# MichSchli/RelationPrediction

Measured on NVIDIA H100. Metric: R-GCN layer fwd+bwd M-edges/sec, higher is better.
Workload: dtype f32

## Files before the change

### relationprediction_b200/csrc/gemm_tf32x3.cu

```cuda
#include <cuda_runtime.h>
#include <stdint.h>

#include <algorithm>
#include <string>

#include "kernels.cuh"

namespace {

constexpr int BM = 128, BN = 128, BK = 32;
constexpr int STAGES = 3;
template <int NST, int TBN>
struct StageShape {
  static constexpr int STAGE_COUNT = NST;
  static constexpr int A_PLANE = BM * BK * 4;
  static constexpr int B_PLANE = TBN * BK * 4;
  static constexpr int BYTES = 2 * A_PLANE + 2 * B_PLANE;
  static constexpr int FRAG = TBN / 2;
};
using NtStage = StageShape<STAGES, BN>;
constexpr int TILE_BYTES = NtStage::A_PLANE;
constexpr int STAGE_BYTES = NtStage::BYTES;
constexpr int SMEM_BYTES = STAGES * STAGE_BYTES + 1024;
constexpr int N_PRODUCERS = 128;
constexpr int N_CONSUMERS = 256;
constexpr int N_THREADS = N_PRODUCERS + N_CONSUMERS;
constexpr int N_FRAG = BN / 2;
static_assert(BM == BN, "the producers use one row schedule for both operands");

__device__ __forceinline__ uint32_t smem_u32(const void* p) {
  return (uint32_t)__cvta_generic_to_shared(p);
}
__device__ __forceinline__ void mbar_init(uint64_t* bar, uint32_t count) {
  asm volatile("mbarrier.init.shared::cta.b64 [%0], %1;" ::"r"(smem_u32(bar)), "r"(count));
}
__device__ __forceinline__ void mbar_arrive(uint64_t* bar) {
  asm volatile("mbarrier.arrive.shared::cta.b64 _, [%0];" ::"r"(smem_u32(bar)) : "memory");
}
__device__ __forceinline__ void mbar_wait(uint64_t* bar, uint32_t parity) {
  asm volatile(
      "{\n\t"
      ".reg .pred p;\n\t"
      "WAIT_LOOP:\n\t"
      "mbarrier.try_wait.parity.shared::cta.b64 p, [%0], %1;\n\t"
      "@p bra WAIT_DONE;\n\t"
      "bra WAIT_LOOP;\n\t"
      "WAIT_DONE:\n\t"
      "}" ::"r"(smem_u32(bar)),
      "r"(parity)
      : "memory");
}
__device__ __forceinline__ void cp_async16(uint32_t dst, const void* src, uint32_t src_bytes) {
  asm volatile("cp.async.cg.shared.global [%0], [%1], 16, %2;" ::"r"(dst), "l"(src), "r"(src_bytes)
               : "memory");
}

__device__ __forceinline__ uint64_t make_desc(uint32_t smem_addr) {
  return (uint64_t)((smem_addr & 0x3FFFFu) >> 4) | (1ull << 16) | ((uint64_t)(1024 >> 4) << 32) | (1ull << 62);
}

__device__ __forceinline__ void wgmma_tf32(float (&d)[64], uint64_t da, uint64_t db, uint32_t accumulate) {
  asm volatile(
      "{\n\t"
      ".reg .pred p;\n\t"
      "setp.ne.b32 p, %66, 0;\n\t"
      "wgmma.mma_async.sync.aligned.m64n128k8.f32.tf32.tf32 "
      "{%0, %1, %2, %3, %4, %5, %6, %7, %8, %9, %10, %11, %12, %13, %14, %15, %16, %17, %18, %19, %20, %21, %22, "
      "%23, %24, %25, %26, %27, %28, %29, %30, %31, %32, %33, %34, %35, %36, %37, %38, %39, %40, %41, %42, %43, %44, "
      "%45, %46, %47, %48, %49, %50, %51, %52, %53, %54, %55, %56, %57, %58, %59, %60, %61, %62, %63}, "
      "%64, %65, p, 1, 1;\n\t"
      "}"
      : "+f"(d[0]), "+f"(d[1]), "+f"(d[2]), "+f"(d[3]), "+f"(d[4]), "+f"(d[5]), "+f"(d[6]), "+f"(d[7]),
        "+f"(d[8]), "+f"(d[9]), "+f"(d[10]), "+f"(d[11]), "+f"(d[12]), "+f"(d[13]), "+f"(d[14]), "+f"(d[15]),
        "+f"(d[16]), "+f"(d[17]), "+f"(d[18]), "+f"(d[19]), "+f"(d[20]), "+f"(d[21]), "+f"(d[22]), "+f"(d[23]),
        "+f"(d[24]), "+f"(d[25]), "+f"(d[26]), "+f"(d[27]), "+f"(d[28]), "+f"(d[29]), "+f"(d[30]), "+f"(d[31]),
        "+f"(d[32]), "+f"(d[33]), "+f"(d[34]), "+f"(d[35]), "+f"(d[36]), "+f"(d[37]), "+f"(d[38]), "+f"(d[39]),
        "+f"(d[40]), "+f"(d[41]), "+f"(d[42]), "+f"(d[43]), "+f"(d[44]), "+f"(d[45]), "+f"(d[46]), "+f"(d[47]),
        "+f"(d[48]), "+f"(d[49]), "+f"(d[50]), "+f"(d[51]), "+f"(d[52]), "+f"(d[53]), "+f"(d[54]), "+f"(d[55]),
        "+f"(d[56]), "+f"(d[57]), "+f"(d[58]), "+f"(d[59]), "+f"(d[60]), "+f"(d[61]), "+f"(d[62]), "+f"(d[63])
      : "l"(da), "l"(db), "r"(accumulate)
      : "memory");
}
__device__ __forceinline__ void wgmma_tf32(float (&d)[32], uint64_t da, uint64_t db, uint32_t accumulate) {
  asm volatile(
      "{\n\t"
      ".reg .pred p;\n\t"
      "setp.ne.b32 p, %34, 0;\n\t"
      "wgmma.mma_async.sync.aligned.m64n64k8.f32.tf32.tf32 "
      "{%0, %1, %2, %3, %4, %5, %6, %7, %8, %9, %10, %11, %12, %13, %14, %15, %16, %17, %18, %19, %20, %21, %22, "
      "%23, %24, %25, %26, %27, %28, %29, %30, %31}, "
      "%32, %33, p, 1, 1;\n\t"
      "}"
      : "+f"(d[0]), "+f"(d[1]), "+f"(d[2]), "+f"(d[3]), "+f"(d[4]), "+f"(d[5]), "+f"(d[6]), "+f"(d[7]),
        "+f"(d[8]), "+f"(d[9]), "+f"(d[10]), "+f"(d[11]), "+f"(d[12]), "+f"(d[13]), "+f"(d[14]), "+f"(d[15]),
        "+f"(d[16]), "+f"(d[17]), "+f"(d[18]), "+f"(d[19]), "+f"(d[20]), "+f"(d[21]), "+f"(d[22]), "+f"(d[23]),
        "+f"(d[24]), "+f"(d[25]), "+f"(d[26]), "+f"(d[27]), "+f"(d[28]), "+f"(d[29]), "+f"(d[30]), "+f"(d[31])
      : "l"(da), "l"(db), "r"(accumulate)
      : "memory");
}
template <int NF>
__device__ __forceinline__ void fence_acc(float (&d)[NF]) {
#pragma unroll
  for (int i = 0; i < NF; ++i) asm volatile("" : "+f"(d[i])::"memory");
}

__device__ __forceinline__ void split_tf32_trunc(float a, float& hi, float& lo) {
  hi = __uint_as_float(__float_as_uint(a) & 0xffffe000u);
  lo = __uint_as_float(__float_as_uint(a - hi) & 0xffffe000u);
}
__device__ __forceinline__ void split_tf32(float a, float& hi, float& lo) {
  uint32_t h, l;
  asm("cvt.rna.tf32.f32 %0, %1;" : "=r"(h) : "f"(a));
  hi = __uint_as_float(h);
  asm("cvt.rna.tf32.f32 %0, %1;" : "=r"(l) : "f"(a - hi));
  lo = __uint_as_float(l);
}

__device__ __forceinline__ uint32_t swz(int r, int c) {
  return (uint32_t)((r >> 3) * 1024 + (r & 7) * 128 + ((c ^ (r & 7)) << 4));
}

template <int NST = STAGES>
__device__ __forceinline__ void init_barriers(uint64_t* full_bar, uint64_t* empty_bar) {
  for (int s = 0; s < NST; ++s) {
    mbar_init(&full_bar[s], N_PRODUCERS);
    mbar_init(&empty_bar[s], N_CONSUMERS);
  }
  asm volatile("fence.mbarrier_init.release.cluster;" ::: "memory");
}

template <class S>
__device__ __forceinline__ void consume_tile(uint32_t smem_base, uint64_t* full_bar, uint64_t* empty_bar, int g0,
                                             int num_kb, uint32_t a_rows, float (&big)[S::FRAG],
                                             float (&small)[S::FRAG]) {
  for (int kb = 0; kb < num_kb; ++kb) {
    const int g = g0 + kb;
    const int s = g % S::STAGE_COUNT;
    mbar_wait(&full_bar[s], (uint32_t)(g / S::STAGE_COUNT) & 1u);
    const uint32_t a_hi = smem_base + s * S::BYTES + a_rows, a_lo = a_hi + S::A_PLANE;
    const uint32_t b_hi = smem_base + s * S::BYTES + 2 * S::A_PLANE, b_lo = b_hi + S::B_PLANE;
    asm volatile("wgmma.fence.sync.aligned;" ::: "memory");
#pragma unroll
    for (int kk = 0; kk < BK / 8; ++kk) {
      const uint64_t dah = make_desc(a_hi + kk * 32), dal = make_desc(a_lo + kk * 32);
      const uint64_t dbh = make_desc(b_hi + kk * 32), dbl = make_desc(b_lo + kk * 32);
      const uint32_t acc = (kb == 0 && kk == 0) ? 0u : 1u;
      wgmma_tf32(small, dal, dbh, acc);
      wgmma_tf32(small, dah, dbl, 1u);
      wgmma_tf32(big, dah, dbh, acc);
    }
    asm volatile("wgmma.commit_group.sync.aligned;" ::: "memory");
    asm volatile("wgmma.wait_group.sync.aligned 0;" ::: "memory");
    fence_acc(big);
    fence_acc(small);
    mbar_arrive(&empty_bar[s]);
  }
}

struct TileCtx {
  int tile;
  int m0, n0;
  int r0, c0;
  int M, N;
  int lane, warp;
};

__device__ __forceinline__ uint32_t col_bit(uint32_t word, int col) { return (word >> (col & 31)) & 1u; }
template <int NF, class Fn>
__device__ __forceinline__ void for_each_col(const TileCtx& t, int h, const uint32_t* bits, int words, Fn fn) {
  const int row = t.r0 + 8 * h;
#pragma unroll
  for (int cb = 0; cb < NF / 16; ++cb) {
    const int chunk = t.n0 + 32 * cb;
    const uint32_t w =
        (bits && row < t.M && chunk < t.N) ? __ldg(bits + (size_t)row * words + (chunk >> 5)) : 0u;
#pragma unroll
    for (int jj = 0; jj < 4; ++jj) {
#pragma unroll
      for (int e = 0; e < 2; ++e) {
        const int j = 4 * cb + jj, col = t.c0 + 8 * j + e;
        fn(4 * j + 2 * h + e, 2 * j + e, col, w);
      }
    }
  }
}
template <class Fn>
__device__ __forceinline__ void for_each_pair(const TileCtx& t, int h, Fn fn) {
#pragma unroll
  for (int j = 0; j < BN / 8; ++j) {
    const int col = t.c0 + 8 * j;
    if (col < t.N) fn(4 * j + 2 * h, col);
  }
}
__device__ __forceinline__ void rank_counts_flush(int raw, int kn, int row, int M, int32_t* raw_cnt,
                                                  int32_t* known_cnt, int lane) {
  raw += __shfl_xor_sync(0xffffffffu, raw, 1);
  raw += __shfl_xor_sync(0xffffffffu, raw, 2);
  kn += __shfl_xor_sync(0xffffffffu, kn, 1);
  kn += __shfl_xor_sync(0xffffffffu, kn, 2);
  if ((lane & 3) == 0 && row < M) {
    if (raw) atomicAdd(raw_cnt + row, raw);
    if (kn) atomicAdd(known_cnt + row, kn);
  }
}
__device__ __forceinline__ void warp_part_store(float x, float* part, const TileCtx& t) {
#pragma unroll
  for (int o = 16; o > 0; o >>= 1) x += __shfl_xor_sync(0xffffffffu, x, o);
  if (t.lane == 0) part[(size_t)t.tile * 8 + t.warp] = x;
}
__device__ __forceinline__ float sigmoid_ref(float x) { return 1.0f / (1.0f + expf(-x)); }

struct StoreEpi {
  float* C;
  int64_t ldc;
  int accumulate;

  __device__ __forceinline__ void operator()(const TileCtx& t, const float (&big)[N_FRAG],
                                             const float (&small)[N_FRAG]) const {
#pragma unroll
    for (int h = 0; h < 2; ++h) {
      const int row = t.r0 + 8 * h;
      if (row >= t.M) continue;
      float* crow = C + (size_t)row * ldc;
      for_each_pair(t, h, [&](int r, int col) {
        float2 o = make_float2(big[r] + small[r], big[r + 1] + small[r + 1]);
        if (accumulate) {
          const float2 old = *reinterpret_cast<const float2*>(crow + col);
          o.x += old.x;
          o.y += old.y;
        }
        *reinterpret_cast<float2*>(crow + col) = o;
      });
    }
  }
};

struct RankEpi {
  const float* gold_sig;
  const int32_t* gold_col;
// ... 137 lines not shown
            bc[h] = oc;
          }
        }
        if (bi >= 0 && bc[h] == mine) left[h] &= ~(1u << bi);
      }
      if (!__any_sync(0xffffffffu, bc[0] != 0x7fffffff || bc[1] != 0x7fffffff)) break;
      if (writer) {
#pragma unroll
        for (int h = 0; h < 2; ++h)
          if (r0 + 8 * h < M)
            *slot(h, p) = bc[h] == 0x7fffffff ? none : make_uint2(__float_as_uint(be[h]), (uint32_t)bc[h]);
      }
    }
    if (writer) {
      for (; p < k; ++p) {
#pragma unroll
        for (int h = 0; h < 2; ++h)
          if (r0 + 8 * h < M) *slot(h, p) = none;
      }
    }
  }
};

struct BceEpi {
  const uint32_t* labels;
  int words;
  float pos, neg;
  float scale;
  const float* g_scale;
  float* Gt;
  int64_t ldgt;
  float* loss_part;

  __device__ __forceinline__ void operator()(const TileCtx& t, const float (&big)[N_FRAG],
                                             const float (&small)[N_FRAG]) const {
    const float gs = scale * (g_scale ? __ldg(g_scale) : 1.f);
    float ls = 0.f;
#pragma unroll
    for (int h = 0; h < 2; ++h) {
      const int row = t.r0 + 8 * h;
      if (row >= t.M) continue;
      for_each_col<N_FRAG>(t, h, labels, words, [&](int r, int, int col, uint32_t word) {
        if (col < t.N) {
          const float z = big[r] + small[r];
          const float y = col_bit(word, col) ? pos : neg;
          ls += fmaxf(z, 0.f) - z * y + log1pf(expf(-fabsf(z)));
          if (Gt) Gt[(size_t)col * ldgt + row] = (1.0f / (1.0f + expf(-z)) - y) * gs;
        }
      });
    }
    warp_part_store(ls, loss_part, t);
  }
};

enum : int { EPI_STORE = 0, EPI_RANK = 1, EPI_HIGHWAY = 2, EPI_VAR = 3, EPI_TOPK = 4, EPI_BCE = 5 };
template <int EPI>
struct Epilogue;
template <> struct Epilogue<EPI_STORE> { using type = StoreEpi; };
template <> struct Epilogue<EPI_RANK> { using type = RankEpi; };
template <> struct Epilogue<EPI_HIGHWAY> { using type = HighwayEpi; };
template <> struct Epilogue<EPI_VAR> { using type = VarEpi; };
template <> struct Epilogue<EPI_TOPK> { using type = TopKEpi; };
template <> struct Epilogue<EPI_BCE> { using type = BceEpi; };

template <int EPI>
__global__ void __launch_bounds__(N_THREADS, 1)
    k_gemm_tf32x3(const float* __restrict__ A, int64_t lda, const float* __restrict__ Bhi,
                  const float* __restrict__ Blo, int64_t ldb, int M, int N, int K, int n_tiles,
                  const typename Epilogue<EPI>::type epi) {
  extern __shared__ uint8_t smem_raw[];
  __shared__ __align__(8) uint64_t full_bar[STAGES], empty_bar[STAGES];

  const uint32_t smem_base = (smem_u32(smem_raw) + 1023u) & ~1023u;
  const int tid = threadIdx.x, lane = tid & 31;
  const int tn = (N + BN - 1) / BN;
  const int num_kb = (K + BK - 1) / BK;
  const int n_mine = (n_tiles - (int)blockIdx.x + (int)gridDim.x - 1) / (int)gridDim.x;
  const int total_g = n_mine * num_kb;

  if (tid == 0) init_barriers(full_bar, empty_bar);
  __syncthreads();

  if (tid < N_PRODUCERS) {
    const int c = tid & 7;
    const int rbase = tid >> 3;
    const uint32_t soff = swz(rbase, c);
    constexpr int NR = BM / 16;

    int b_kb = 0, b_tile = (int)blockIdx.x, b_stage = 0;
    size_t b_off = 0;
    uint32_t b_ok = 0;
    auto b_set_tile = [&]() {
      const int r0 = (b_tile % tn) * BN + rbase;
      b_ok = 0;
#pragma unroll
      for (int i = 0; i < NR; ++i) b_ok |= (r0 + 16 * i < N ? 1u : 0u) << i;
      b_off = (b_ok & 1u) ? (size_t)r0 * ldb + c * 4 : 0;
    };
    b_set_tile();
    auto issue_b = [&]() {
      const uint32_t b_hi = smem_base + b_stage * STAGE_BYTES + 2 * TILE_BYTES + soff, b_lo = b_hi + TILE_BYTES;
      const bool col_ok = b_kb * BK + c * 4 < K;
      const size_t kof = b_off + (size_t)b_kb * BK;
#pragma unroll
      for (int i = 0; i < NR; ++i) {
        const bool ok = col_ok && ((b_ok >> i) & 1u);
        const size_t o = kof + (size_t)(16 * i) * ldb;
        cp_async16(b_hi + 2048 * i, ok ? Bhi + o : Bhi, ok ? 16u : 0u);
        cp_async16(b_lo + 2048 * i, ok ? Blo + o : Blo, ok ? 16u : 0u);
      }
      asm volatile("cp.async.commit_group;" ::: "memory");
      b_stage = b_stage + 1 == STAGES ? 0 : b_stage + 1;
      if (++b_kb == num_kb) {
        b_kb = 0;
        b_tile += (int)gridDim.x;
        b_set_tile();
      }
    };
    int a_kb = 0, a_tile = (int)blockIdx.x;
    size_t a_off = 0;
    uint32_t a_ok = 0;
    auto a_set_tile = [&]() {
      const int r0 = (a_tile / tn) * BM + rbase;
      a_ok = 0;
#pragma unroll
      for (int i = 0; i < NR; ++i) a_ok |= (r0 + 16 * i < M ? 1u : 0u) << i;
      a_off = (a_ok & 1u) ? (size_t)r0 * lda + c * 4 : 0;
    };
    a_set_tile();
    auto load_a = [&](float4 (&v)[NR]) {
      const bool col_ok = a_kb * BK + c * 4 < K;
      const float* p = A + a_off + (size_t)a_kb * BK;
#pragma unroll
      for (int i = 0; i < NR; ++i)
        v[i] = (col_ok && ((a_ok >> i) & 1u)) ? __ldg(reinterpret_cast<const float4*>(p + (size_t)(16 * i) * lda))
                                               : make_float4(0.f, 0.f, 0.f, 0.f);
      if (++a_kb == num_kb) {
        a_kb = 0;
        a_tile += (int)gridDim.x;
        a_set_tile();
      }
    };
    constexpr int PF = 2;
    float4 vbuf[PF + 1][NR];
    mbar_wait(&empty_bar[0], 1u);
    issue_b();
    for (int p = 0; p < PF; ++p)
      if (p < total_g) load_a(vbuf[p]);
    int s = 0;
    uint32_t ph_next = 0;
    for (int g0 = 0; g0 < total_g; g0 += PF + 1) {
#pragma unroll
      for (int u = 0; u <= PF; ++u) {
        const int g = g0 + u;
        if (g >= total_g) break;
        const bool more = g + 1 < total_g;
        const int s1 = s + 1 == STAGES ? 0 : s + 1;
        if (s1 == 0) ph_next ^= 1u;
        if (more) {
          mbar_wait(&empty_bar[s1], ph_next ^ 1u);
          issue_b();
        }
        if (g + PF < total_g) load_a(vbuf[(u + PF) % (PF + 1)]);
        const uint32_t a_hi = smem_base + s * STAGE_BYTES + soff, a_lo = a_hi + TILE_BYTES;
#pragma unroll
        for (int i = 0; i < NR; ++i) {
          float4 hi, lo;
          split_tf32_trunc(vbuf[u][i].x, hi.x, lo.x);
          split_tf32_trunc(vbuf[u][i].y, hi.y, lo.y);
          split_tf32_trunc(vbuf[u][i].z, hi.z, lo.z);
          split_tf32_trunc(vbuf[u][i].w, hi.w, lo.w);
          asm volatile("st.shared.v4.f32 [%0], {%1, %2, %3, %4};" ::"r"(a_hi + 2048 * i), "f"(hi.x), "f"(hi.y),
                       "f"(hi.z), "f"(hi.w)
                       : "memory");
          asm volatile("st.shared.v4.f32 [%0], {%1, %2, %3, %4};" ::"r"(a_lo + 2048 * i), "f"(lo.x), "f"(lo.y),
                       "f"(lo.z), "f"(lo.w)
                       : "memory");
        }
        if (more)
          asm volatile("cp.async.wait_group 1;" ::: "memory");
        else
          asm volatile("cp.async.wait_group 0;" ::: "memory");
        asm volatile("fence.proxy.async.shared::cta;" ::: "memory");
        mbar_arrive(&full_bar[s]);
        s = s1;
      }
    }
  } else {
    const int ctid = tid - N_PRODUCERS;
    const int wg = ctid >> 7, warp = ctid >> 5;
    const uint32_t a_rows = (uint32_t)(wg * 64 * 128);
    float big[N_FRAG], small[N_FRAG];
    for (int ti = 0; ti < n_mine; ++ti) {
      const int tile = (int)blockIdx.x + ti * (int)gridDim.x;
      const int m0 = (tile / tn) * BM, n0 = (tile % tn) * BN;
      consume_tile<NtStage>(smem_base, full_bar, empty_bar, ti * num_kb, num_kb, a_rows, big, small);
      const int r0 = m0 + wg * 64 + (warp & 3) * 16 + (lane >> 2), c0 = n0 + 2 * (lane & 3);
      const TileCtx t{tile, m0, n0, r0, c0, M, N, lane, warp};
      epi(t, big, small);
    }
  }
}

constexpr int TN_FLUSH_KB = 32;
constexpr int TN_STAGES = 2;
using TnStage = StageShape<TN_STAGES, BN>;
constexpr int TN_RAW = 3;
constexpr int RAW_TILE_BYTES = BK * BM * 4;
constexpr int RAW_BYTES = 2 * RAW_TILE_BYTES;
constexpr int TN_SMEM_BYTES = TN_STAGES * STAGE_BYTES + TN_RAW * RAW_BYTES + 1024;
static_assert(TN_SMEM_BYTES <= 227 * 1024, "TN kernel exceeds the shared memory of a block");
static_assert(N_PRODUCERS == 128 && BK == 32 && BM == 128, "the TN producer's lane mapping assumes these");

__device__ __forceinline__ float4 ld_shared_v4(uint32_t addr) {
  float4 v;
  asm volatile("ld.shared.v4.f32 {%0, %1, %2, %3}, [%4];" : "=f"(v.x), "=f"(v.y), "=f"(v.z), "=f"(v.w) : "r"(addr)
               : "memory");
  return v;
}
__device__ __forceinline__ void st_shared_v4(uint32_t addr, float x, float y, float z, float w) {
  asm volatile("st.shared.v4.f32 [%0], {%1, %2, %3, %4};" ::"r"(addr), "f"(x), "f"(y), "f"(z), "f"(w) : "memory");
}

__global__ void __launch_bounds__(N_THREADS, 1)
    k_gemm_tn_tf32x3(const float* __restrict__ A, int64_t lda, const float* __restrict__ B, int64_t ldb,
                     float* __restrict__ C, int64_t ldc, int M, int N, int K, int kb_per_split) {
  extern __shared__ uint8_t smem_raw[];
  __shared__ __align__(8) uint64_t full_bar[TN_STAGES], empty_bar[TN_STAGES];
  const uint32_t smem_base = (smem_u32(smem_raw) + 1023u) & ~1023u;
  const int tid = threadIdx.x, warp = tid >> 5, lane = tid & 31;
  const int tm = (M + BM - 1) / BM, tiles = tm * ((N + BN - 1) / BN);
  const int tile = (int)blockIdx.x % tiles, split = (int)blockIdx.x / tiles;
  const int m0 = (tile % tm) * BM, n0 = (tile / tm) * BN;
  const int kb_begin = split * kb_per_split;
  const int num_kb = min(kb_per_split, (K + BK - 1) / BK - kb_begin);

  if (tid == 0) init_barriers<TN_STAGES>(full_bar, empty_bar);
  __syncthreads();

  if (tid < N_PRODUCERS) {
    const uint32_t raw_base = smem_base + TN_STAGES * STAGE_BYTES;
    const bool a_ok = m0 + 4 * lane < M, b_ok = n0 + 4 * lane < N;
    const float* pa = A + (a_ok ? m0 + 4 * lane : 0);
    const float* pb = B + (b_ok ? n0 + 4 * lane : 0);
    auto issue = [&](int kbi) {
      const uint32_t dst = raw_base + (kbi % TN_RAW) * RAW_BYTES;
      const int k0 = (kb_begin + kbi) * BK + warp;
#pragma unroll
      for (int i = 0; i < 8; ++i) {
        const bool kok = k0 + 4 * i < K;
        const size_t row = kok ? (size_t)(k0 + 4 * i) : 0;
        const uint32_t off = (uint32_t)((warp + 4 * i) * 512 + ((lane ^ i) << 4));
        cp_async16(dst + off, pa + row * lda, kok && a_ok ? 16u : 0u);
        cp_async16(dst + RAW_TILE_BYTES + off, pb + row * ldb, kok && b_ok ? 16u : 0u);
      }
      asm volatile("cp.async.commit_group;" ::: "memory");
    };
    const int g = lane & 7;
    auto convert = [&](uint32_t raw, uint32_t hi_plane) {
#pragma unroll
      for (int u = 0; u < 2; ++u) {
        const int h = (lane >> 3) + 4 * warp + 16 * u;
        float4 v[4];
#pragma unroll
        for (int j = 0; j < 4; ++j) v[j] = ld_shared_v4(raw + (4 * g + j) * 512 + ((h ^ g) << 4));
        const float x[4][4] = {{v[0].x, v[1].x, v[2].x, v[3].x}, {v[0].y, v[1].y, v[2].y, v[3].y},
                               {v[0].z, v[1].z, v[2].z, v[3].z}, {v[0].w, v[1].w, v[2].w, v[3].w}};
#pragma unroll
        for (int i = 0; i < 4; ++i) {
          float hi[4], lo[4];
#pragma unroll
          for (int j = 0; j < 4; ++j) split_tf32_trunc(x[i][j], hi[j], lo[j]);
          const uint32_t a = hi_plane + swz(4 * h + i, g);
          st_shared_v4(a, hi[0], hi[1], hi[2], hi[3]);
          st_shared_v4(a + TILE_BYTES, lo[0], lo[1], lo[2], lo[3]);
        }
      }
    };
    issue(0);
    if (num_kb > 1)
      issue(1);
    else
      asm volatile("cp.async.commit_group;" ::: "memory");
    for (int kb = 0; kb < num_kb; ++kb) {
      asm volatile("cp.async.wait_group 1;" ::: "memory");
      asm volatile("bar.sync 1, %0;" ::"n"(N_PRODUCERS) : "memory");
      if (kb + 2 < num_kb)
        issue(kb + 2);
      else
        asm volatile("cp.async.commit_group;" ::: "memory");
      const int s = kb % TN_STAGES;
      mbar_wait(&empty_bar[s], ((uint32_t)(kb / TN_STAGES) & 1u) ^ 1u);
      const uint32_t raw = raw_base + (kb % TN_RAW) * RAW_BYTES, stage = smem_base + s * STAGE_BYTES;
      convert(raw, stage);
      convert(raw + RAW_TILE_BYTES, stage + 2 * TILE_BYTES);
      asm volatile("fence.proxy.async.shared::cta;" ::: "memory");
      mbar_arrive(&full_bar[s]);
    }
  } else {
    const int ctid = tid - N_PRODUCERS;
    const int wg = ctid >> 7;
    const int r0 = m0 + wg * 64 + ((ctid >> 5) & 3) * 16 + (lane >> 2);
    const int c0 = n0 + 2 * (lane & 3);
    float* const cbase = C + (size_t)r0 * ldc + c0;
    float big[N_FRAG], small[N_FRAG];
    for (int kc = 0; kc < num_kb; kc += TN_FLUSH_KB) {
      consume_tile<TnStage>(smem_base, full_bar, empty_bar, kc, min(TN_FLUSH_KB, num_kb - kc),
                            (uint32_t)(wg * 64 * 128), big, small);
      float* cp = cbase;
      asm volatile("" : "+l"(cp));
#pragma unroll
      for (int h = 0; h < 2; ++h) {
        if (r0 + 8 * h >= M) continue;
        float* crow = cp + (size_t)(8 * h) * ldc;
#pragma unroll
        for (int j = 0; j < BN / 8; ++j) {
          if (c0 + 8 * j < N)
            asm volatile("red.global.add.v2.f32 [%0], {%1, %2};" ::"l"(crow + 8 * j),
                         "f"(big[4 * j + 2 * h] + small[4 * j + 2 * h]),
                         "f"(big[4 * j + 2 * h + 1] + small[4 * j + 2 * h + 1])
                         : "memory");
        }
      }
    }
  }
}

__global__ void k_split_b(const float* __restrict__ B, int64_t ldb, int N, int K, int transposed,
                          float* __restrict__ hi, float* __restrict__ lo) {
  const int64_t total = (int64_t)N * K;
  for (int64_t i = blockIdx.x * (int64_t)blockDim.x + threadIdx.x; i < total;
       i += (int64_t)gridDim.x * blockDim.x) {
    const int n = (int)(i / K), k = (int)(i % K);
    const float v = transposed ? __ldg(B + (size_t)k * ldb + n) : __ldg(B + (size_t)n * ldb + k);
    float h, l;
    split_tf32(v, h, l);
    hi[i] = h;
    lo[i] = l;
  }
}

__global__ void k_split_b_interleave(const float* __restrict__ Wmu, const float* __restrict__ Wsig, int d, int w,
                                     int transposed, float* __restrict__ hi, float* __restrict__ lo) {
  const int64_t total = (int64_t)2 * d * w;
  const int K = transposed ? d : 2 * w;
  for (int64_t i = blockIdx.x * (int64_t)blockDim.x + threadIdx.x; i < total;
       i += (int64_t)gridDim.x * blockDim.x) {
    const int n = (int)(i / K), k = (int)(i % K);
    const int row = transposed ? k : n, c = transposed ? n : k;
    const float v = __ldg(((c & 1) ? Wsig : Wmu) + (size_t)row * w + (c >> 1));
    float h, l;
    split_tf32(v, h, l);
    hi[i] = h;
    lo[i] = l;
  }
}

constexpr int EN_BN = 64;
constexpr int EN_STAGES = 4;
constexpr int EN_LOOKAHEAD = 2;
using EnsStage = StageShape<EN_STAGES, EN_BN>;
constexpr int EN_Q_BYTES = EnsStage::A_PLANE;
constexpr int EN_C_BYTES = EnsStage::B_PLANE;
constexpr int EN_STAGE_BYTES = EnsStage::BYTES;
constexpr int EN_SMEM_BYTES = EN_STAGES * EN_STAGE_BYTES + 1024;
constexpr int EN_FRAG = EnsStage::FRAG;
static_assert(EN_SMEM_BYTES <= 227 * 1024, "ensemble kernel exceeds the shared memory of a block");
static_assert(EN_LOOKAHEAD < EN_STAGES, "the lookahead needs a free stage");

struct EnsMember {
  const float* q_hi;
  const float* q_lo;
  const float* c_hi;
  const float* c_lo;
  const float* gold_sig;
  int K;
};
struct EnsEpi {
  EnsMember a, b;
  double w, omw;
  const int32_t* gold_col;
  const uint32_t* known;
  int words;
  int32_t* raw_cnt;
  int32_t* known_cnt;
};

__global__ void __launch_bounds__(N_THREADS, 1)
    k_gemm_ensemble_rank(int M, int N, int n_tiles, EnsEpi re) {
  extern __shared__ uint8_t smem_raw[];
  __shared__ __align__(8) uint64_t full_bar[EN_STAGES], empty_bar[EN_STAGES];
  const uint32_t smem_base = (smem_u32(smem_raw) + 1023u) & ~1023u;
  const int tid = threadIdx.x, lane = tid & 31;
  const int tn = (N + EN_BN - 1) / EN_BN;
  const int nkb_a = (re.a.K + BK - 1) / BK, nkb_b = (re.b.K + BK - 1) / BK, nkb = nkb_a + nkb_b;
  const int n_mine = (n_tiles - (int)blockIdx.x + (int)gridDim.x - 1) / (int)gridDim.x;
  const int total_g = n_mine * nkb;

  if (tid == 0) init_barriers<EN_STAGES>(full_bar, empty_bar);
  __syncthreads();

  if (tid < N_PRODUCERS) {
    const int c = tid & 7;
    const int rbase = tid >> 3;
    const uint32_t soff = swz(rbase, c);
    int i_tile = (int)blockIdx.x, i_kb = 0, stage = 0;
    auto issue = [&]() {
      const bool mb = i_kb >= nkb_a;
      const float* qh = mb ? re.b.q_hi : re.a.q_hi;
      const float* ql = mb ? re.b.q_lo : re.a.q_lo;
      const float* ch = mb ? re.b.c_hi : re.a.c_hi;
      const float* cl = mb ? re.b.c_lo : re.a.c_lo;
      const int K = mb ? re.b.K : re.a.K;
      const int k = (mb ? i_kb - nkb_a : i_kb) * BK + c * 4;
      const bool col_ok = k < K;
      const int m0 = (i_tile / tn) * BM, n0 = (i_tile % tn) * EN_BN;
      const uint32_t st = smem_base + stage * EN_STAGE_BYTES + soff;
#pragma unroll
      for (int i = 0; i < BM / 16; ++i) {
        const int row = m0 + rbase + 16 * i;
        const bool ok = col_ok && row < M;
        const size_t o = ok ? (size_t)row * K + k : 0;
        cp_async16(st + 2048 * i, qh + o, ok ? 16u : 0u);
        cp_async16(st + EN_Q_BYTES + 2048 * i, ql + o, ok ? 16u : 0u);
      }
#pragma unroll
      for (int i = 0; i < EN_BN / 16; ++i) {
        const int row = n0 + rbase + 16 * i;
        const bool ok = col_ok && row < N;
        const size_t o = ok ? (size_t)row * K + k : 0;
        cp_async16(st + 2 * EN_Q_BYTES + 2048 * i, ch + o, ok ? 16u : 0u);
        cp_async16(st + 2 * EN_Q_BYTES + EN_C_BYTES + 2048 * i, cl + o, ok ? 16u : 0u);
      }
      asm volatile("cp.async.commit_group;" ::: "memory");
      stage = stage + 1 == EN_STAGES ? 0 : stage + 1;
      if (++i_kb == nkb) {
        i_kb = 0;
        i_tile += (int)gridDim.x;
      }
    };
    for (int g = 0; g < EN_LOOKAHEAD; ++g) {
      if (g < total_g) {
        mbar_wait(&empty_bar[g % EN_STAGES], ((uint32_t)(g / EN_STAGES) & 1u) ^ 1u);
        issue();
      } else {
        asm volatile("cp.async.commit_group;" ::: "memory");
      }
    }
    for (int g = 0; g < total_g; ++g) {
      const int gn = g + EN_LOOKAHEAD;
      if (gn < total_g) {
        mbar_wait(&empty_bar[gn % EN_STAGES], ((uint32_t)(gn / EN_STAGES) & 1u) ^ 1u);
        issue();
      } else {
        asm volatile("cp.async.commit_group;" ::: "memory");
      }
      asm volatile("cp.async.wait_group %0;" ::"n"(EN_LOOKAHEAD) : "memory");
      asm volatile("fence.proxy.async.shared::cta;" ::: "memory");
      mbar_arrive(&full_bar[g % EN_STAGES]);
    }
  } else {
    const int ctid = tid - N_PRODUCERS;
    const int wg = ctid >> 7, warp = ctid >> 5;
    const uint32_t a_rows = (uint32_t)(wg * 64 * 128);
    float big_a[EN_FRAG], small_a[EN_FRAG], big_b[EN_FRAG], small_b[EN_FRAG];
    for (int ti = 0; ti < n_mine; ++ti) {
      const int tile = (int)blockIdx.x + ti * (int)gridDim.x;
      const int m0 = (tile / tn) * BM, n0 = (tile % tn) * EN_BN;
      consume_tile<EnsStage>(smem_base, full_bar, empty_bar, ti * nkb, nkb_a, a_rows, big_a, small_a);
      consume_tile<EnsStage>(smem_base, full_bar, empty_bar, ti * nkb + nkb_a, nkb_b, a_rows, big_b, small_b);
      const int r0 = m0 + wg * 64 + (warp & 3) * 16 + (lane >> 2), c0 = n0 + 2 * (lane & 3);
      const TileCtx t{tile, m0, n0, r0, c0, M, N, lane, warp};
#pragma unroll
      for (int h = 0; h < 2; ++h) {
        const int row = t.r0 + 8 * h;
        int raw = 0, kn = 0;
        if (row < M) {
          const double G = __dadd_rn(__dmul_rn(re.w, (double)__ldg(re.a.gold_sig + row)),
                                     __dmul_rn(re.omw, (double)__ldg(re.b.gold_sig + row)));
          const int gold_c = __ldg(re.gold_col + row);
          for_each_col<EN_FRAG>(t, h, re.known, re.words, [&](int r, int, int col, uint32_t word) {
            const float sa = sigmoid_ref(big_a[r] + small_a[r]);
            const float sb = sigmoid_ref(big_b[r] + small_b[r]);
            const double cv = __dadd_rn(__dmul_rn(re.w, (double)sa), __dmul_rn(re.omw, (double)sb));
            if (col < N && (cv >= G || col == gold_c)) {
              ++raw;
              kn += (int)col_bit(word, col);
            }
          });
        }
        rank_counts_flush(raw, kn, row, M, re.raw_cnt, re.known_cnt, lane);
      }
    }
  }
}

__global__ void k_split_trunc(float* __restrict__ a, float* __restrict__ lo, int64_t count4) {
  for (int64_t i = blockIdx.x * (int64_t)blockDim.x + threadIdx.x; i < count4; i += (int64_t)gridDim.x * blockDim.x) {
    float4 v = reinterpret_cast<float4*>(a)[i], h, l;
    split_tf32_trunc(v.x, h.x, l.x);
    split_tf32_trunc(v.y, h.y, l.y);
    split_tf32_trunc(v.z, h.z, l.z);
    split_tf32_trunc(v.w, h.w, l.w);
    reinterpret_cast<float4*>(a)[i] = h;
    reinterpret_cast<float4*>(lo)[i] = l;
  }
}

}

static int sm_count() {
  int dev = 0, sms = 132;
  cudaGetDevice(&dev);
  cudaDeviceGetAttribute(&sms, cudaDevAttrMultiProcessorCount, dev);
  return sms;
}

static int64_t tiles_of(int64_t M, int64_t N, int bn) { return ((M + BM - 1) / BM) * ((N + bn - 1) / bn); }

template <auto Kernel, class... Args>
static int launch_persistent(const char* what, const char* label, int smem, int64_t tiles, int64_t tile_limit,
                             cudaStream_t st, Args... args) {
  static bool attr_set = false;
  if (!attr_set) {
    int rc = rgcn_check_cuda(cudaFuncSetAttribute(Kernel, cudaFuncAttributeMaxDynamicSharedMemorySize, smem),
                             (std::string("cudaFuncSetAttribute(") + label + " smem)").c_str());
    if (rc) return rc;
    attr_set = true;
  }
  if (tiles > tile_limit) {
    rgcn_set_error(std::string(what) + ": too many tiles");
    return RGCN_ERR_INVALID;
  }
  const unsigned grid = (unsigned)std::min<int64_t>(tiles, sm_count());
  Kernel<<<grid, N_THREADS, smem, st>>>(args...);
  ++g_rgcn_launches;
  return rgcn_check_cuda(cudaGetLastError(), label);
}
constexpr int64_t TILE_LIMIT = 0x7fffffffLL;
constexpr int64_t PART_TILE_LIMIT = TILE_LIMIT / 8;

template <int EPI>
static int launch_nt(const char* what, const char* label, int64_t tile_limit, cudaStream_t st, const float* A,
                     int64_t lda, const float* Bt_hi, const float* Bt_lo, int64_t ldb, int M, int N, int K,
                     const typename Epilogue<EPI>::type& epi) {
  const int64_t tiles = tiles_of(M, N, BN);
  return launch_persistent<k_gemm_tf32x3<EPI>>(what, label, SMEM_BYTES, tiles, tile_limit, st, A, lda, Bt_hi, Bt_lo,
                                               ldb, M, N, K, (int)tiles, epi);
}

static int split_blocks(int64_t items) { return (int)std::min<int64_t>((items + 255) / 256, 132 * 8); }

int launch_gemm_split_b(const float* B, int64_t ldb, int N, int K, int transposed, float* hi, float* lo,
// ... 163 lines not shown
```

Baseline: 129.2.

## Feed WGMMA A operand from registers with consumer-side split and deeper pipelining

```diff
diff --git a/relationprediction_b200/csrc/gemm_tf32x3.cu b/relationprediction_b200/csrc/gemm_tf32x3.cu
--- a/relationprediction_b200/csrc/gemm_tf32x3.cu
+++ b/relationprediction_b200/csrc/gemm_tf32x3.cu
@@ -9,24 +9,28 @@
 namespace {
 
 constexpr int BM = 128, BN = 128, BK = 32;
-constexpr int STAGES = 3;
-template <int NST, int TBN>
+constexpr int STAGES = 4;
+template <int NST, int TBN, int A_PLANES>
 struct StageShape {
   static constexpr int STAGE_COUNT = NST;
   static constexpr int A_PLANE = BM * BK * 4;
+  static constexpr int A_BYTES = A_PLANES * A_PLANE;
   static constexpr int B_PLANE = TBN * BK * 4;
-  static constexpr int BYTES = 2 * A_PLANE + 2 * B_PLANE;
+  static constexpr int BYTES = A_BYTES + 2 * B_PLANE;
   static constexpr int FRAG = TBN / 2;
 };
-using NtStage = StageShape<STAGES, BN>;
+using NtStage = StageShape<STAGES, BN, 1>;
 constexpr int TILE_BYTES = NtStage::A_PLANE;
 constexpr int STAGE_BYTES = NtStage::BYTES;
 constexpr int SMEM_BYTES = STAGES * STAGE_BYTES + 1024;
+static_assert(SMEM_BYTES <= 227 * 1024, "NT kernel exceeds the shared memory of a block");
 constexpr int N_PRODUCERS = 128;
 constexpr int N_CONSUMERS = 256;
 constexpr int N_THREADS = N_PRODUCERS + N_CONSUMERS;
 constexpr int N_FRAG = BN / 2;
-static_assert(BM == BN, "the producers use one row schedule for both operands");
+constexpr int NT_PRODUCER_REGS = 40, TN_PRODUCER_REGS = 56;
+template <int PRODUCER_REGS>
+constexpr int CONSUMER_REGS = (168 * N_THREADS - N_PRODUCERS * PRODUCER_REGS) / N_CONSUMERS / 8 * 8;
 
 __device__ __forceinline__ uint32_t smem_u32(const void* p) {
   return (uint32_t)__cvta_generic_to_shared(p);
@@ -59,16 +63,16 @@
   return (uint64_t)((smem_addr & 0x3FFFFu) >> 4) | (1ull << 16) | ((uint64_t)(1024 >> 4) << 32) | (1ull << 62);
 }
 
-__device__ __forceinline__ void wgmma_tf32(float (&d)[64], uint64_t da, uint64_t db, uint32_t accumulate) {
+__device__ __forceinline__ void wgmma_tf32(float (&d)[64], const uint32_t (&a)[4], uint64_t db, uint32_t accumulate) {
   asm volatile(
       "{\n\t"
       ".reg .pred p;\n\t"
-      "setp.ne.b32 p, %66, 0;\n\t"
+      "setp.ne.b32 p, %69, 0;\n\t"
       "wgmma.mma_async.sync.aligned.m64n128k8.f32.tf32.tf32 "
       "{%0, %1, %2, %3, %4, %5, %6, %7, %8, %9, %10, %11, %12, %13, %14, %15, %16, %17, %18, %19, %20, %21, %22, "
       "%23, %24, %25, %26, %27, %28, %29, %30, %31, %32, %33, %34, %35, %36, %37, %38, %39, %40, %41, %42, %43, %44, "
       "%45, %46, %47, %48, %49, %50, %51, %52, %53, %54, %55, %56, %57, %58, %59, %60, %61, %62, %63}, "
-      "%64, %65, p, 1, 1;\n\t"
+      "{%64, %65, %66, %67}, %68, p, 1, 1;\n\t"
       "}"
       : "+f"(d[0]), "+f"(d[1]), "+f"(d[2]), "+f"(d[3]), "+f"(d[4]), "+f"(d[5]), "+f"(d[6]), "+f"(d[7]),
         "+f"(d[8]), "+f"(d[9]), "+f"(d[10]), "+f"(d[11]), "+f"(d[12]), "+f"(d[13]), "+f"(d[14]), "+f"(d[15]),
@@ -78,24 +82,24 @@
         "+f"(d[40]), "+f"(d[41]), "+f"(d[42]), "+f"(d[43]), "+f"(d[44]), "+f"(d[45]), "+f"(d[46]), "+f"(d[47]),
         "+f"(d[48]), "+f"(d[49]), "+f"(d[50]), "+f"(d[51]), "+f"(d[52]), "+f"(d[53]), "+f"(d[54]), "+f"(d[55]),
         "+f"(d[56]), "+f"(d[57]), "+f"(d[58]), "+f"(d[59]), "+f"(d[60]), "+f"(d[61]), "+f"(d[62]), "+f"(d[63])
-      : "l"(da), "l"(db), "r"(accumulate)
+      : "r"(a[0]), "r"(a[1]), "r"(a[2]), "r"(a[3]), "l"(db), "r"(accumulate)
       : "memory");
 }
-__device__ __forceinline__ void wgmma_tf32(float (&d)[32], uint64_t da, uint64_t db, uint32_t accumulate) {
+__device__ __forceinline__ void wgmma_tf32(float (&d)[32], const uint32_t (&a)[4], uint64_t db, uint32_t accumulate) {
   asm volatile(
       "{\n\t"
       ".reg .pred p;\n\t"
-      "setp.ne.b32 p, %34, 0;\n\t"
+      "setp.ne.b32 p, %37, 0;\n\t"
       "wgmma.mma_async.sync.aligned.m64n64k8.f32.tf32.tf32 "
       "{%0, %1, %2, %3, %4, %5, %6, %7, %8, %9, %10, %11, %12, %13, %14, %15, %16, %17, %18, %19, %20, %21, %22, "
       "%23, %24, %25, %26, %27, %28, %29, %30, %31}, "
-      "%32, %33, p, 1, 1;\n\t"
+      "{%32, %33, %34, %35}, %36, p, 1, 1;\n\t"
       "}"
       : "+f"(d[0]), "+f"(d[1]), "+f"(d[2]), "+f"(d[3]), "+f"(d[4]), "+f"(d[5]), "+f"(d[6]), "+f"(d[7]),
         "+f"(d[8]), "+f"(d[9]), "+f"(d[10]), "+f"(d[11]), "+f"(d[12]), "+f"(d[13]), "+f"(d[14]), "+f"(d[15]),
         "+f"(d[16]), "+f"(d[17]), "+f"(d[18]), "+f"(d[19]), "+f"(d[20]), "+f"(d[21]), "+f"(d[22]), "+f"(d[23]),
         "+f"(d[24]), "+f"(d[25]), "+f"(d[26]), "+f"(d[27]), "+f"(d[28]), "+f"(d[29]), "+f"(d[30]), "+f"(d[31])
-      : "l"(da), "l"(db), "r"(accumulate)
+      : "r"(a[0]), "r"(a[1]), "r"(a[2]), "r"(a[3]), "l"(db), "r"(accumulate)
       : "memory");
 }
 template <int NF>
@@ -129,32 +133,88 @@
   asm volatile("fence.mbarrier_init.release.cluster;" ::: "memory");
 }
 
-template <class S>
+template <int PRODUCER_REGS>
+__device__ __forceinline__ void producer_regs() {
+  asm volatile("setmaxnreg.dec.sync.aligned.u32 %0;" ::"n"(PRODUCER_REGS));
+}
+template <int PRODUCER_REGS>
+__device__ __forceinline__ void consumer_regs() {
+  asm volatile("setmaxnreg.inc.sync.aligned.u32 %0;" ::"n"(CONSUMER_REGS<PRODUCER_REGS>));
+}
+
+__device__ __forceinline__ float ld_shared_f32(uint32_t addr) {
+  float v;
+  asm volatile("ld.shared.f32 %0, [%1];" : "=f"(v) : "r"(addr) : "memory");
+  return v;
+}
+
+using FragA = uint32_t[BK / 8][4];
+
+template <bool PRESPLIT>
+struct KMajorA {
+  uint32_t off;
+
+  __device__ __forceinline__ KMajorA(int wg, int warp, int lane)
+      : off(swz(wg * 64 + 16 * (warp & 3) + (lane >> 2), 0) + 4 * (lane & 3)) {}
+  __device__ __forceinline__ void operator()(uint32_t stage, FragA& hi, FragA& lo) const {
+#pragma unroll
+    for (int kk = 0; kk < BK / 8; ++kk)
+#pragma unroll
+      for (int r = 0; r < 4; ++r) {
+        const uint32_t a = (stage + off + 1024 * (r & 1)) ^ (uint32_t)((2 * kk + (r >> 1)) << 4);
+        if (PRESPLIT) {
+          hi[kk][r] = __float_as_uint(ld_shared_f32(a));
+          lo[kk][r] = __float_as_uint(ld_shared_f32(a + BM * BK * 4));
+        } else {
+          float h, l;
+          split_tf32_trunc(ld_shared_f32(a), h, l);
+          hi[kk][r] = __float_as_uint(h);
+          lo[kk][r] = __float_as_uint(l);
+        }
+      }
+  }
+};
+
+template <class S, bool FENCE, class LoadA>
+__device__ __forceinline__ void consume_block(uint32_t smem_base, uint64_t* full_bar, uint64_t* empty_bar, int g0,
+                                              int kb, const LoadA& load_a, FragA& a_hi, FragA& a_lo,
+                                              float (&big)[S::FRAG], float (&small)[S::FRAG]) {
+  const int g = g0 + kb;
+  const int s = g % S::STAGE_COUNT;
+  mbar_wait(&full_bar[s], (uint32_t)(g / S::STAGE_COUNT) & 1u);
+  if (FENCE) asm volatile("fence.proxy.async.shared::cta;" ::: "memory");
+  const uint32_t stage = smem_base + s * S::BYTES;
+  load_a(stage, a_hi, a_lo);
+  const uint32_t b_hi = stage + S::A_BYTES, b_lo = b_hi + S::B_PLANE;
+  const uint64_t dbh0 = make_desc(b_hi), dbl0 = make_desc(b_lo);
+  asm volatile("wgmma.fence.sync.aligned;" ::: "memory");
+#pragma unroll
+  for (int kk = 0; kk < BK / 8; ++kk) {
+    const uint64_t dbh = dbh0 + 2 * kk, dbl = dbl0 + 2 * kk;
+    const uint32_t acc = (kb == 0 && kk == 0) ? 0u : 1u;
+    wgmma_tf32(small, a_lo[kk], dbh, acc);
+    wgmma_tf32(small, a_hi[kk], dbl, 1u);
+    wgmma_tf32(big, a_hi[kk], dbh, acc);
+  }
+  asm volatile("wgmma.commit_group.sync.aligned;" ::: "memory");
+  asm volatile("wgmma.wait_group.sync.aligned 1;" ::: "memory");
+  if (kb > 0) mbar_arrive(&empty_bar[(g - 1) % S::STAGE_COUNT]);
+}
+
+template <class S, bool FENCE, class LoadA>
 __device__ __forceinline__ void consume_tile(uint32_t smem_base, uint64_t* full_bar, uint64_t* empty_bar, int g0,
-                                             int num_kb, uint32_t a_rows, float (&big)[S::FRAG],
+                                             int num_kb, const LoadA& load_a, float (&big)[S::FRAG],
                                              float (&small)[S::FRAG]) {
-  for (int kb = 0; kb < num_kb; ++kb) {
-    const int g = g0 + kb;
-    const int s = g % S::STAGE_COUNT;
-    mbar_wait(&full_bar[s], (uint32_t)(g / S::STAGE_COUNT) & 1u);
-    const uint32_t a_hi = smem_base + s * S::BYTES + a_rows, a_lo = a_hi + S::A_PLANE;
-    const uint32_t b_hi = smem_base + s * S::BYTES + 2 * S::A_PLANE, b_lo = b_hi + S::B_PLANE;
-    asm volatile("wgmma.fence.sync.aligned;" ::: "memory");
-#pragma unroll
-    for (int kk = 0; kk < BK / 8; ++kk) {
-      const uint64_t dah = make_desc(a_hi + kk * 32), dal = make_desc(a_lo + kk * 32);
-      const uint64_t dbh = make_desc(b_hi + kk * 32), dbl = make_desc(b_lo + kk * 32);
-      const uint32_t acc = (kb == 0 && kk == 0) ? 0u : 1u;
-      wgmma_tf32(small, dal, dbh, acc);
-      wgmma_tf32(small, dah, dbl, 1u);
-      wgmma_tf32(big, dah, dbh, acc);
-    }
-    asm volatile("wgmma.commit_group.sync.aligned;" ::: "memory");
-    asm volatile("wgmma.wait_group.sync.aligned 0;" ::: "memory");
-    fence_acc(big);
-    fence_acc(small);
-    mbar_arrive(&empty_bar[s]);
-  }
+  FragA hi0, lo0, hi1, lo1;
+  for (int kb = 0; kb < num_kb; kb += 2) {
+    consume_block<S, FENCE>(smem_base, full_bar, empty_bar, g0, kb, load_a, hi0, lo0, big, small);
+    if (kb + 1 < num_kb)
+      consume_block<S, FENCE>(smem_base, full_bar, empty_bar, g0, kb + 1, load_a, hi1, lo1, big, small);
+  }
+  asm volatile("wgmma.wait_group.sync.aligned 0;" ::: "memory");
+  fence_acc(big);
+  fence_acc(small);
+  mbar_arrive(&empty_bar[(g0 + num_kb - 1) % S::STAGE_COUNT]);
 }
 
 struct TileCtx {
@@ -458,119 +518,53 @@
   __syncthreads();
 
   if (tid < N_PRODUCERS) {
+    producer_regs<NT_PRODUCER_REGS>();
     const int c = tid & 7;
     const int rbase = tid >> 3;
     const uint32_t soff = swz(rbase, c);
-    constexpr int NR = BM / 16;
-
-    int b_kb = 0, b_tile = (int)blockIdx.x, b_stage = 0;
-    size_t b_off = 0;
-    uint32_t b_ok = 0;
-    auto b_set_tile = [&]() {
-      const int r0 = (b_tile % tn) * BN + rbase;
-      b_ok = 0;
-#pragma unroll
-      for (int i = 0; i < NR; ++i) b_ok |= (r0 + 16 * i < N ? 1u : 0u) << i;
-      b_off = (b_ok & 1u) ? (size_t)r0 * ldb + c * 4 : 0;
+    int i_tile = (int)blockIdx.x, i_kb = 0, stage = 0;
+    auto issue = [&]() {
+      const int k = i_kb * BK + c * 4;
+      const bool col_ok = k < K;
+      const int m0 = (i_tile / tn) * BM, n0 = (i_tile % tn) * BN;
+      const uint32_t st = smem_base + stage * STAGE_BYTES + soff;
+#pragma unroll
+      for (int i = 0; i < BM / 16; ++i) {
+        const int row = m0 + rbase + 16 * i;
+        const bool ok = col_ok && row < M;
+        cp_async16(st + 2048 * i, ok ? A + (size_t)row * lda + k : A, ok ? 16u : 0u);
+      }
+#pragma unroll
+      for (int i = 0; i < BN / 16; ++i) {
+        const int row = n0 + rbase + 16 * i;
+        const bool ok = col_ok && row < N;
+        const size_t o = ok ? (size_t)row * ldb + k : 0;
+        cp_async16(st + TILE_BYTES + 2048 * i, Bhi + o, ok ? 16u : 0u);
+        cp_async16(st + 2 * TILE_BYTES + 2048 * i, Blo + o, ok ? 16u : 0u);
+      }
+      stage = stage + 1 == STAGES ? 0 : stage + 1;
+      if (++i_kb == num_kb) {
+        i_kb = 0;
+        i_tile += (int)gridDim.x;
+      }
     };
-    b_set_tile();
-    auto issue_b = [&]() {
-      const uint32_t b_hi = smem_base + b_stage * STAGE_BYTES + 2 * TILE_BYTES + soff, b_lo = b_hi + TILE_BYTES;
-      const bool col_ok = b_kb * BK + c * 4 < K;
-      const size_t kof = b_off + (size_t)b_kb * BK;
-#pragma unroll
-      for (int i = 0; i < NR; ++i) {
-        const bool ok = col_ok && ((b_ok >> i) & 1u);
-        const size_t o = kof + (size_t)(16 * i) * ldb;
-        cp_async16(b_hi + 2048 * i, ok ? Bhi + o : Bhi, ok ? 16u : 0u);
-        cp_async16(b_lo + 2048 * i, ok ? Blo + o : Blo, ok ? 16u : 0u);
-      }
-      asm volatile("cp.async.commit_group;" ::: "memory");
-      b_stage = b_stage + 1 == STAGES ? 0 : b_stage + 1;
-      if (++b_kb == num_kb) {
-        b_kb = 0;
-        b_tile += (int)gridDim.x;
-        b_set_tile();
-      }
-    };
-    int a_kb = 0, a_tile = (int)blockIdx.x;
-    size_t a_off = 0;
-    uint32_t a_ok = 0;
-    auto a_set_tile = [&]() {
-      const int r0 = (a_tile / tn) * BM + rbase;
-      a_ok = 0;
-#pragma unroll
-      for (int i = 0; i < NR; ++i) a_ok |= (r0 + 16 * i < M ? 1u : 0u) << i;
-      a_off = (a_ok & 1u) ? (size_t)r0 * lda + c * 4 : 0;
-    };
-    a_set_tile();
-    auto load_a = [&](float4 (&v)[NR]) {
-      const bool col_ok = a_kb * BK + c * 4 < K;
-      const float* p = A + a_off + (size_t)a_kb * BK;
-#pragma unroll
-      for (int i = 0; i < NR; ++i)
-        v[i] = (col_ok && ((a_ok >> i) & 1u)) ? __ldg(reinterpret_cast<const float4*>(p + (size_t)(16 * i) * lda))
-                                               : make_float4(0.f, 0.f, 0.f, 0.f);
-      if (++a_kb == num_kb) {
-        a_kb = 0;
-        a_tile += (int)gridDim.x;
-        a_set_tile();
-      }
-    };
-    constexpr int PF = 2;
-    float4 vbuf[PF + 1][NR];
-    mbar_wait(&empty_bar[0], 1u);
-    issue_b();
-    for (int p = 0; p < PF; ++p)
-      if (p < total_g) load_a(vbuf[p]);
-    int s = 0;
-    uint32_t ph_next = 0;
-    for (int g0 = 0; g0 < total_g; g0 += PF + 1) {
-#pragma unroll
-      for (int u = 0; u <= PF; ++u) {
-        const int g = g0 + u;
-        if (g >= total_g) break;
-        const bool more = g + 1 < total_g;
-        const int s1 = s + 1 == STAGES ? 0 : s + 1;
-        if (s1 == 0) ph_next ^= 1u;
-        if (more) {
-          mbar_wait(&empty_bar[s1], ph_next ^ 1u);
-          issue_b();
-        }
-        if (g + PF < total_g) load_a(vbuf[(u + PF) % (PF + 1)]);
-        const uint32_t a_hi = smem_base + s * STAGE_BYTES + soff, a_lo = a_hi + TILE_BYTES;
-#pragma unroll
-        for (int i = 0; i < NR; ++i) {
-          float4 hi, lo;
-          split_tf32_trunc(vbuf[u][i].x, hi.x, lo.x);
-          split_tf32_trunc(vbuf[u][i].y, hi.y, lo.y);
-          split_tf32_trunc(vbuf[u][i].z, hi.z, lo.z);
-          split_tf32_trunc(vbuf[u][i].w, hi.w, lo.w);
-          asm volatile("st.shared.v4.f32 [%0], {%1, %2, %3, %4};" ::"r"(a_hi + 2048 * i), "f"(hi.x), "f"(hi.y),
-                       "f"(hi.z), "f"(hi.w)
-                       : "memory");
-          asm volatile("st.shared.v4.f32 [%0], {%1, %2, %3, %4};" ::"r"(a_lo + 2048 * i), "f"(lo.x), "f"(lo.y),
-                       "f"(lo.z), "f"(lo.w)
-                       : "memory");
-        }
-        if (more)
-          asm volatile("cp.async.wait_group 1;" ::: "memory");
-        else
-          asm volatile("cp.async.wait_group 0;" ::: "memory");
-        asm volatile("fence.proxy.async.shared::cta;" ::: "memory");
-        mbar_arrive(&full_bar[s]);
-        s = s1;
-      }
-    }
+    for (int g = 0; g < total_g; ++g) {
+      mbar_wait(&empty_bar[g % STAGES], ((uint32_t)(g / STAGES) & 1u) ^ 1u);
+      issue();
+      asm volatile("cp.async.mbarrier.arrive.noinc.shared::cta.b64 [%0];" ::"r"(smem_u32(&full_bar[g % STAGES]))
+                   : "memory");
+    }
+    asm volatile("cp.async.wait_all;" ::: "memory");
   } else {
+    consumer_regs<NT_PRODUCER_REGS>();
     const int ctid = tid - N_PRODUCERS;
     const int wg = ctid >> 7, warp = ctid >> 5;
-    const uint32_t a_rows = (uint32_t)(wg * 64 * 128);
+    const KMajorA<false> load_a(wg, warp, lane);
     float big[N_FRAG], small[N_FRAG];
     for (int ti = 0; ti < n_mine; ++ti) {
       const int tile = (int)blockIdx.x + ti * (int)gridDim.x;
       const int m0 = (tile / tn) * BM, n0 = (tile % tn) * BN;
-      consume_tile<NtStage>(smem_base, full_bar, empty_bar, ti * num_kb, num_kb, a_rows, big, small);
+      consume_tile<NtStage, true>(smem_base, full_bar, empty_bar, ti * num_kb, num_kb, load_a, big, small);
       const int r0 = m0 + wg * 64 + (warp & 3) * 16 + (lane >> 2), c0 = n0 + 2 * (lane & 3);
       const TileCtx t{tile, m0, n0, r0, c0, M, N, lane, warp};
       epi(t, big, small);
@@ -579,14 +573,40 @@
 }
 
 constexpr int TN_FLUSH_KB = 32;
-constexpr int TN_STAGES = 2;
-using TnStage = StageShape<TN_STAGES, BN>;
-constexpr int TN_RAW = 3;
-constexpr int RAW_TILE_BYTES = BK * BM * 4;
-constexpr int RAW_BYTES = 2 * RAW_TILE_BYTES;
-constexpr int TN_SMEM_BYTES = TN_STAGES * STAGE_BYTES + TN_RAW * RAW_BYTES + 1024;
+constexpr int TN_STAGES = 4;
+using TnStage = StageShape<TN_STAGES, BN, 1>;
+constexpr int TN_RAW = 2;
+constexpr int TN_LOOKAHEAD = 2;
+constexpr int RAW_TILE_BYTES = BK * BN * 4;
+constexpr int TN_SMEM_BYTES = TN_STAGES * STAGE_BYTES + TN_RAW * RAW_TILE_BYTES + 1024;
 static_assert(TN_SMEM_BYTES <= 227 * 1024, "TN kernel exceeds the shared memory of a block");
 static_assert(N_PRODUCERS == 128 && BK == 32 && BM == 128, "the TN producer's lane mapping assumes these");
+static_assert(TN_LOOKAHEAD == TN_STAGES - 2, "block kb + TN_LOOKAHEAD refills the MMA stage of block kb - 2");
+static_assert(TN_LOOKAHEAD == TN_RAW, "block kb + TN_LOOKAHEAD refills the staging block of block kb");
+
+struct TnRawA {
+  uint32_t off[2];
+
+  __device__ __forceinline__ TnRawA(int wg, int warp, int lane) {
+    const int t = lane & 3;
+#pragma unroll
+    for (int h = 0; h < 2; ++h) {
+      const int m = wg * 64 + 16 * (warp & 3) + (lane >> 2) + 8 * h;
+      off[h] = (uint32_t)(t * 512 + (((m >> 2) ^ (2 * t)) << 4) + 4 * (m & 3));
+    }
+  }
+  __device__ __forceinline__ void operator()(uint32_t stage, FragA& hi, FragA& lo) const {
+#pragma unroll
+    for (int kk = 0; kk < BK / 8; ++kk)
+#pragma unroll
+      for (int r = 0; r < 4; ++r) {
+        float h, l;
+        split_tf32_trunc(ld_shared_f32(stage + off[r & 1] + 512 * (8 * kk + 4 * (r >> 1))), h, l);
+        hi[kk][r] = __float_as_uint(h);
+        lo[kk][r] = __float_as_uint(l);
+      }
+  }
+};
 
 __device__ __forceinline__ float4 ld_shared_v4(uint32_t addr) {
   float4 v;
@@ -615,20 +635,21 @@
   __syncthreads();
 
   if (tid < N_PRODUCERS) {
+    producer_regs<TN_PRODUCER_REGS>();
     const uint32_t raw_base = smem_base + TN_STAGES * STAGE_BYTES;
     const bool a_ok = m0 + 4 * lane < M, b_ok = n0 + 4 * lane < N;
     const float* pa = A + (a_ok ? m0 + 4 * lane : 0);
     const float* pb = B + (b_ok ? n0 + 4 * lane : 0);
     auto issue = [&](int kbi) {
-      const uint32_t dst = raw_base + (kbi % TN_RAW) * RAW_BYTES;
+      const uint32_t dst_a = smem_base + (kbi % TN_STAGES) * STAGE_BYTES + warp * 512 + ((lane ^ (2 * warp)) << 4);
+      const uint32_t dst_b = raw_base + (kbi % TN_RAW) * RAW_TILE_BYTES + warp * 512;
       const int k0 = (kb_begin + kbi) * BK + warp;
 #pragma unroll
       for (int i = 0; i < 8; ++i) {
         const bool kok = k0 + 4 * i < K;
         const size_t row = kok ? (size_t)(k0 + 4 * i) : 0;
-        const uint32_t off = (uint32_t)((warp + 4 * i) * 512 + ((lane ^ i) << 4));
-        cp_async16(dst + off, pa + row * lda, kok && a_ok ? 16u : 0u);
-        cp_async16(dst + RAW_TILE_BYTES + off, pb + row * ldb, kok && b_ok ? 16u : 0u);
+        cp_async16(dst_a + 2048 * i, pa + row * lda, kok && a_ok ? 16u : 0u);
+        cp_async16(dst_b + 2048 * i + ((lane ^ i) << 4), pb + row * ldb, kok && b_ok ? 16u : 0u);
       }
       asm volatile("cp.async.commit_group;" ::: "memory");
     };
@@ -653,36 +674,39 @@
         }
       }
     };
-    issue(0);
-    if (num_kb > 1)
-      issue(1);
-    else
-      asm volatile("cp.async.commit_group;" ::: "memory");
-    for (int kb = 0; kb < num_kb; ++kb) {
-      asm volatile("cp.async.wait_group 1;" ::: "memory");
-      asm volatile("bar.sync 1, %0;" ::"n"(N_PRODUCERS) : "memory");
-      if (kb + 2 < num_kb)
-        issue(kb + 2);
+    for (int p = 0; p < TN_LOOKAHEAD; ++p) {
+      if (p < num_kb)
+        issue(p);
       else
         asm volatile("cp.async.commit_group;" ::: "memory");
+    }
+    for (int kb = 0; kb < num_kb; ++kb) {
+      asm volatile("cp.async.wait_group %0;" ::"n"(TN_LOOKAHEAD - 1) : "memory");
+      asm volatile("bar.sync 1, %0;" ::"n"(N_PRODUCERS) : "memory");
       const int s = kb % TN_STAGES;
-      mbar_wait(&empty_bar[s], ((uint32_t)(kb / TN_STAGES) & 1u) ^ 1u);
-      const uint32_t raw = raw_base + (kb % TN_RAW) * RAW_BYTES, stage = smem_base + s * STAGE_BYTES;
-      convert(raw, stage);
-      convert(raw + RAW_TILE_BYTES, stage + 2 * TILE_BYTES);
+      convert(raw_base + (kb % TN_RAW) * RAW_TILE_BYTES, smem_base + s * STAGE_BYTES + TILE_BYTES);
       asm volatile("fence.proxy.async.shared::cta;" ::: "memory");
       mbar_arrive(&full_bar[s]);
+      const int kn = kb + TN_LOOKAHEAD;
+      if (kn < num_kb) {
+        asm volatile("bar.sync 1, %0;" ::"n"(N_PRODUCERS) : "memory");
+        mbar_wait(&empty_bar[kn % TN_STAGES], ((uint32_t)(kn / TN_STAGES) & 1u) ^ 1u);
+        issue(kn);
+      } else {
+        asm volatile("cp.async.commit_group;" ::: "memory");
+      }
     }
   } else {
+    consumer_regs<TN_PRODUCER_REGS>();
     const int ctid = tid - N_PRODUCERS;
     const int wg = ctid >> 7;
     const int r0 = m0 + wg * 64 + ((ctid >> 5) & 3) * 16 + (lane >> 2);
     const int c0 = n0 + 2 * (lane & 3);
     float* const cbase = C + (size_t)r0 * ldc + c0;
+    const TnRawA load_a(wg, ctid >> 5, lane);
     float big[N_FRAG], small[N_FRAG];
     for (int kc = 0; kc < num_kb; kc += TN_FLUSH_KB) {
-      consume_tile<TnStage>(smem_base, full_bar, empty_bar, kc, min(TN_FLUSH_KB, num_kb - kc),
-                            (uint32_t)(wg * 64 * 128), big, small);
+      consume_tile<TnStage, false>(smem_base, full_bar, empty_bar, kc, min(TN_FLUSH_KB, num_kb - kc), load_a, big, small);
       float* cp = cbase;
       asm volatile("" : "+l"(cp));
 #pragma unroll
@@ -735,7 +759,7 @@
 constexpr int EN_BN = 64;
 constexpr int EN_STAGES = 4;
 constexpr int EN_LOOKAHEAD = 2;
-using EnsStage = StageShape<EN_STAGES, EN_BN>;
+using EnsStage = StageShape<EN_STAGES, EN_BN, 2>;
 constexpr int EN_Q_BYTES = EnsStage::A_PLANE;
 constexpr int EN_C_BYTES = EnsStage::B_PLANE;
 constexpr int EN_STAGE_BYTES = EnsStage::BYTES;
@@ -777,6 +801,7 @@
   __syncthreads();
 
   if (tid < N_PRODUCERS) {
+    producer_regs<NT_PRODUCER_REGS>();
     const int c = tid & 7;
     const int rbase = tid >> 3;
     const uint32_t soff = swz(rbase, c);
@@ -836,15 +861,16 @@
       mbar_arrive(&full_bar[g % EN_STAGES]);
     }
   } else {
+    consumer_regs<NT_PRODUCER_REGS>();
     const int ctid = tid - N_PRODUCERS;
     const int wg = ctid >> 7, warp = ctid >> 5;
-    const uint32_t a_rows = (uint32_t)(wg * 64 * 128);
+    const KMajorA<true> load_a(wg, warp, lane);
     float big_a[EN_FRAG], small_a[EN_FRAG], big_b[EN_FRAG], small_b[EN_FRAG];
     for (int ti = 0; ti < n_mine; ++ti) {
       const int tile = (int)blockIdx.x + ti * (int)gridDim.x;
       const int m0 = (tile / tn) * BM, n0 = (tile % tn) * EN_BN;
-      consume_tile<EnsStage>(smem_base, full_bar, empty_bar, ti * nkb, nkb_a, a_rows, big_a, small_a);
-      consume_tile<EnsStage>(smem_base, full_bar, empty_bar, ti * nkb + nkb_a, nkb_b, a_rows, big_b, small_b);
+      consume_tile<EnsStage, false>(smem_base, full_bar, empty_bar, ti * nkb, nkb_a, load_a, big_a, small_a);
+      consume_tile<EnsStage, false>(smem_base, full_bar, empty_bar, ti * nkb + nkb_a, nkb_b, load_a, big_b, small_b);
       const int r0 = m0 + wg * 64 + (warp & 3) * 16 + (lane >> 2), c0 = n0 + 2 * (lane & 3);
       const TileCtx t{tile, m0, n0, r0, c0, M, N, lane, warp};
 #pragma unroll
```

Result: faster. 132.3, median of 6 (+2.4%).
